# claudiotomasi/LearnMultigrid

Measured on AMD Instinct MI355X. Metric: fine-level DoF*sweeps/s, 2-D Poisson V-cycle, higher is better.
Workload: dtype f64; 1 GPU; 2-D structured P1 Poisson 4096x4096 elements (16785409 DoF, 83861509 nnz, CSR fp64/int32), 6-level V(3,3) cycle, weighted Jacobi omega=0.80, tensor-product geometric transfer, Galerkin RAP by device SpGEMM; mode=vcycle, step=one full V-cycle, hipgraph=True, partition=row blocks of grid lines over 1 rank(s), sweep_variant=0, packed_csr=True, fine_level_format=stencil, problem=poisson, transfer=geometric

## Files before the change

### include/lmg.h

```cpp
#ifndef LMG_H
#define LMG_H

#include <stddef.h>
#include <stdint.h>

#ifdef __cplusplus
extern "C" {
#endif

#define LMG_VERSION 100

typedef enum {
    LMG_OK = 0,
    LMG_ERR_ARG = -1,
    LMG_ERR_ALIGN = -2,
    LMG_ERR_LAUNCH = -3,
    LMG_ERR_CAPACITY = -4,
    LMG_ERR_NODEVICE = -5
} lmg_status;

int lmg_version(void);
const char *lmg_status_string(int status);
int lmg_device_count(void);

// ... 17 lines not shown
int lmg_pcsr_tile_rows(void);
int lmg_pcsr_sweep(int mode, int64_t n, int64_t nnz, int32_t tile_rows, int32_t tile_cap,
                   const int32_t *d_tile_base,
                   const int32_t *d_tile_colbase, const uint8_t *d_rowlen, const void *d_col,
                   int colmode, const void *d_val, int valmode, const double *d_dict, int32_t ndict,
                   const double *d_x, const double *d_b, double *d_out, double alpha, double beta,
                   double *d_partials, double *d_norm2, void *stream);

int lmg_rpat_limits(int32_t *max_patterns, int32_t *max_entries);
int lmg_rpat_sweep(int mode, int64_t n, const uint8_t *d_pid, int32_t npat, int32_t nent, int32_t max_len,
                   const int32_t *d_pat_ptr, const int32_t *d_pat_off, const double *d_pat_val,
                   const double *d_x, const double *d_b, double *d_out, double alpha, double beta,
                   double *d_partials, double *d_norm2, void *stream);
int lmg_rpat_row_hash(int64_t n, const int32_t *d_rowptr, const int32_t *d_colidx, const double *d_vals,
                      uint64_t *d_hash, void *stream);
int lmg_rpat_claim(int64_t n, const uint8_t *d_pid, int32_t *d_rep, void *stream);
int lmg_rpat_verify(int64_t n, int64_t ncols, const int32_t *d_rowptr, const int32_t *d_colidx,
                    const double *d_vals, const uint8_t *d_pid, int32_t npat, const int32_t *d_pat_ptr,
                    const int32_t *d_pat_off, const double *d_pat_val, int32_t *d_mismatch, void *stream);

int lmg_rpat_sweep_grid(int mode, int64_t n, const int32_t *h_grid_map, const uint8_t *d_pid, int32_t npat,
                        int32_t nent, int32_t max_len, const int32_t *d_pat_ptr, const int32_t *d_pat_off,
                        const double *d_pat_val, const double *d_x, const double *d_b, double *d_out,
                        double alpha, double beta, double *d_partials, double *d_norm2, void *stream);
int lmg_rpat_row_hash_grid(int64_t n, const int32_t *h_grid_map, const int32_t *d_rowptr,
                           const int32_t *d_colidx, const double *d_vals, uint64_t *d_hash, void *stream);
int lmg_rpat_verify_grid(int64_t n, int64_t ncols, const int32_t *h_grid_map, const int32_t *d_rowptr,
                         const int32_t *d_colidx, const double *d_vals, const uint8_t *d_pid, int32_t npat,
                         const int32_t *d_pat_ptr, const int32_t *d_pat_off, const double *d_pat_val,
                         int32_t *d_mismatch, void *stream);

int lmg_stencil_limits(int32_t *max_patterns);
int lmg_stencil_sweep(int mode, int64_t n, int32_t line_stride, const uint8_t *d_pid, int32_t npat,
                      const double *d_st_val, const int32_t *d_st_mask, uint32_t union_mask, const double *d_x,
                      const double *d_b, double *d_out, double alpha, double beta, double *d_partials,
                      double *d_norm2, void *stream);

int lmg_stencil_smooth_supported(uint32_t union_mask);
int lmg_stencil_smooth(int64_t n, int32_t line_stride, const uint8_t *d_pid, int32_t npat,
                       const double *d_st_val, const int32_t *d_st_mask, uint32_t union_mask,
                       int32_t hot_pattern, const double *h_hot_val, int sweeps, const double *d_x_in,
                       const double *d_b, double omega, double *d_x_out, double *d_r_out, void *stream);

int lmg_stencil_smooth_tiled_supported(uint32_t union_mask);
int lmg_stencil_smooth_tiled(int64_t n, int32_t line_stride, const uint8_t *d_pid, int32_t npat,
                             const double *d_st_val, const int32_t *d_st_mask, uint32_t union_mask,
                             int32_t hot_pattern, const double *h_hot_val, int sweeps, const double *d_x_in,
                             const double *d_b, double omega, double *d_x_out, double *d_r_out, void *stream);
int lmg_stencil_smooth_tiled_prolong(int64_t n, int32_t line_stride, const uint8_t *d_pid, int32_t npat,
                                     const double *d_st_val, const int32_t *d_st_mask, uint32_t union_mask,
                                     int32_t hot_pattern, const double *h_hot_val, int sweeps, const double *d_x_in,
                                     const double *d_b, double omega, double *d_x_out, int64_t n_coarse,
                                     int32_t coarse_stride, const double *d_e_coarse, const uint8_t *d_p_pid,
                                     int32_t p_npat, const double *d_p_val, const int32_t *d_p_mask, void *stream);
int lmg_stencil_smooth_tiled_restrict(int64_t n, int32_t line_stride, const uint8_t *d_pid, int32_t npat,
                                      const double *d_st_val, const int32_t *d_st_mask, uint32_t union_mask,
                                      int32_t hot_pattern, const double *h_hot_val, int sweeps, const double *d_x_in,
                                      const double *d_b, double omega, double *d_x_out, int64_t n_coarse,
                                      int32_t coarse_stride, double *d_b_coarse, const uint8_t *d_r_pid,
                                      int32_t r_npat, const double *d_r_val, const int32_t *d_r_mask, void *stream);

int lmg_dia_smooth_supported(uint32_t union_mask);
int lmg_dia_fill(int64_t n, int32_t line_stride, const int32_t *d_rowptr, const int32_t *d_colidx, const double *d_vals,
                 uint32_t union_mask, double *d_dia, int32_t *d_mismatch, uint32_t *d_mask_out, void *stream);
int lmg_dia_smooth(int64_t n, int32_t line_stride, uint32_t union_mask, const double *d_dia, int sweeps,
                   const double *d_x_in, const double *d_b, double omega, double *d_x_out, double *d_r_out, void *stream);

int lmg_stencil_smooth_prolong_supported(uint32_t union_mask);
int lmg_stencil_smooth_prolong(int64_t n, int32_t line_stride, const uint8_t *d_pid, int32_t npat,
                               const double *d_st_val, const int32_t *d_st_mask, uint32_t union_mask,
                               int32_t hot_pattern, const double *h_hot_val, int sweeps, const double *d_x_in,
                               const double *d_b, double omega, double *d_x_out, int64_t n_coarse,
                               int32_t coarse_stride, const double *d_e_coarse, const uint8_t *d_p_pid,
                               int32_t p_npat, const double *d_p_val, const int32_t *d_p_mask,
                               const int32_t *h_hot_pairs, const double *h_hot_pval, void *stream);

int lmg_stencil_smooth_restrict(int64_t n, int32_t line_stride, const uint8_t *d_pid, int32_t npat,
                                const double *d_st_val, const int32_t *d_st_mask, uint32_t union_mask,
                                int32_t hot_pattern, const double *h_hot_val, int sweeps, const double *d_x_in,
                                const double *d_b, double omega, double *d_x_out, int64_t n_coarse,
                                int32_t coarse_stride, double *d_b_coarse, const uint8_t *d_r_pid,
                                int32_t r_npat, const double *d_r_val, const int32_t *d_r_mask, int32_t hot_r,
                                const double *h_hot_rval, void *stream);

int lmg_sell_sweep(int mode, int64_t n, const int64_t *d_slice_base, const int32_t *d_slice_len,
                   const int32_t *d_slice_cmin, const int32_t *d_rowlen, const void *d_col, int colmode,
                   const double *d_val, int32_t max_len, const double *d_x, const double *d_b, double *d_out,
                   double alpha, double beta, double *d_partials, double *d_norm2, void *stream);
int lmg_sell_slice_info(int64_t n, const int32_t *d_rowptr, const int32_t *d_colidx, int32_t *d_slice_len,
                        int32_t *d_cmin, int32_t *d_cmax, void *stream);
int lmg_sell_fill(int64_t n, const int32_t *d_rowptr, const int32_t *d_colidx, const double *d_vals,
                  const int64_t *d_slice_base, const int32_t *d_slice_cmin, int colmode, void *d_col_out,
                  double *d_val_out, void *stream);

int lmg_pcsr_tile_colrange(int64_t n, int32_t tile_rows, const int32_t *d_rowptr, const int32_t *d_colidx,
                           int32_t *d_cmin, int32_t *d_cmax, void *stream);
int lmg_pcsr_encode_cols16(int64_t n, int32_t tile_rows, const int32_t *d_rowptr, const int32_t *d_colidx,
                           const int32_t *d_colbase, uint16_t *d_out, void *stream);
int lmg_value_set_collect(const uint64_t *d_table, int64_t table_slots, uint64_t *d_out, int32_t cap, int32_t *d_count,
                          void *stream);
int lmg_value_set_insert(int64_t count, const double *d_vals, uint64_t *d_table, int64_t table_slots,
                         int32_t limit, int32_t *d_state, void *stream);
int lmg_value_encode(int64_t count, const double *d_vals, const double *d_dict, int32_t ndict, int width,
                     void *d_out, int32_t *d_missing, void *stream);
int lmg_csr_inverse_diagonal(int64_t n, const int32_t *d_rowptr, const int32_t *d_colidx, const double *d_vals,
                             double *d_dinv, void *stream);

int lmg_csr_transpose_max_row(void);
int lmg_csr_transpose_count(int64_t nnz, int64_t ncols, const int32_t *d_colidx, int32_t *d_counts, void *stream);
int lmg_csr_transpose_fill(int64_t n, int64_t ncols, const int32_t *d_rowptr, const int32_t *d_colidx,
                           const double *d_vals, const int32_t *d_t_rowptr, int32_t *d_cursor, int32_t *d_t_colidx,
                           double *d_t_vals, void *stream);

// ... 130 lines not shown
```

### learnmultigrid_amd/_lib.py

```python
import ctypes
import os
import subprocess

import torch

_HERE = os.path.dirname(os.path.abspath(__file__))
LIB_PATH = os.environ.get("LMG_LIB_PATH") or os.path.join(_HERE, "liblmg_hip.so")
CSRC = os.path.join(_HERE, "csrc")

_c = ctypes
_i64, _i32, _f64, _p, _cp = _c.c_int64, _c.c_int32, _c.c_double, _c.c_void_p, _c.c_char_p

SIGNATURES = {
    "lmg_version": (_c.c_int, []),
    "lmg_status_string": (_cp, [_c.c_int]),
    "lmg_device_count": (_c.c_int, []),
    "lmg_tune_set": (_c.c_int, [_cp, _c.c_int]),
    "lmg_tune_get": (_c.c_int, [_cp]),
    "lmg_partials_count": (_i64, [_i64]),
    "lmg_csr_residual_norm2": (_c.c_int, [_i64, _i64, _p, _p, _p, _p, _p, _p, _p, _p, _p]),
    "lmg_csr_jacobi": (_c.c_int, [_i64, _i64, _p, _p, _p, _p, _p, _f64, _p, _p]),
    "lmg_csr_spmv": (_c.c_int, [_i64, _i64, _p, _p, _p, _p, _p, _f64, _f64, _p]),
    "lmg_pcsr_tile_rows": (_c.c_int, []),
    "lmg_pcsr_sweep": (_c.c_int, [_c.c_int, _i64, _i64, _i32, _i32, _p, _p, _p, _p, _c.c_int, _p, _c.c_int, _p, _i32,
                                  _p, _p, _p, _f64, _f64, _p, _p, _p]),
    "lmg_rpat_limits": (_c.c_int, [_p, _p]),
    "lmg_rpat_sweep": (_c.c_int, [_c.c_int, _i64, _p, _i32, _i32, _i32, _p, _p, _p, _p, _p, _p, _f64, _f64, _p, _p, _p]),
    "lmg_rpat_row_hash": (_c.c_int, [_i64, _p, _p, _p, _p, _p]),
    "lmg_rpat_claim": (_c.c_int, [_i64, _p, _p, _p]),
    "lmg_rpat_verify": (_c.c_int, [_i64, _i64, _p, _p, _p, _p, _i32, _p, _p, _p, _p, _p]),
    "lmg_rpat_sweep_grid": (_c.c_int, [_c.c_int, _i64, _p, _p, _i32, _i32, _i32, _p, _p, _p, _p, _p, _p, _f64, _f64, _p, _p, _p]),
    "lmg_rpat_row_hash_grid": (_c.c_int, [_i64, _p, _p, _p, _p, _p, _p]),
    "lmg_rpat_verify_grid": (_c.c_int, [_i64, _i64, _p, _p, _p, _p, _p, _i32, _p, _p, _p, _p, _p]),
    "lmg_stencil_limits": (_c.c_int, [_p]),
    "lmg_stencil_sweep": (_c.c_int, [_c.c_int, _i64, _i32, _p, _i32, _p, _p, _c.c_uint32, _p, _p, _p, _f64, _f64, _p, _p, _p]),
    "lmg_stencil_smooth_supported": (_c.c_int, [_c.c_uint32]),
    "lmg_stencil_smooth": (_c.c_int, [_i64, _i32, _p, _i32, _p, _p, _c.c_uint32, _i32, _p, _c.c_int, _p, _p, _f64, _p, _p, _p]),
    "lmg_stencil_smooth_tiled_supported": (_c.c_int, [_c.c_uint32]),
    "lmg_stencil_smooth_tiled": (_c.c_int, [_i64, _i32, _p, _i32, _p, _p, _c.c_uint32, _i32, _p, _c.c_int, _p, _p, _f64, _p, _p, _p]),
    "lmg_stencil_smooth_tiled_prolong": (_c.c_int, [_i64, _i32, _p, _i32, _p, _p, _c.c_uint32, _i32, _p, _c.c_int, _p, _p, _f64, _p,
                                                    _i64, _i32, _p, _p, _i32, _p, _p, _p]),
    "lmg_stencil_smooth_tiled_restrict": (_c.c_int, [_i64, _i32, _p, _i32, _p, _p, _c.c_uint32, _i32, _p, _c.c_int, _p, _p, _f64, _p,
                                                     _i64, _i32, _p, _p, _i32, _p, _p, _p]),
    "lmg_dia_smooth_supported": (_c.c_int, [_c.c_uint32]),
    "lmg_dia_fill": (_c.c_int, [_i64, _i32, _p, _p, _p, _c.c_uint32, _p, _p, _p, _p]),
    "lmg_dia_smooth": (_c.c_int, [_i64, _i32, _c.c_uint32, _p, _c.c_int, _p, _p, _f64, _p, _p, _p]),
    "lmg_stencil_smooth_prolong_supported": (_c.c_int, [_c.c_uint32]),
    "lmg_stencil_smooth_prolong": (_c.c_int, [_i64, _i32, _p, _i32, _p, _p, _c.c_uint32, _i32, _p, _c.c_int, _p, _p, _f64, _p,
                                              _i64, _i32, _p, _p, _i32, _p, _p, _p, _p, _p]),
    "lmg_stencil_smooth_restrict": (_c.c_int, [_i64, _i32, _p, _i32, _p, _p, _c.c_uint32, _i32, _p, _c.c_int, _p, _p, _f64, _p,
                                               _i64, _i32, _p, _p, _i32, _p, _p, _i32, _p, _p]),
    "lmg_sell_sweep": (_c.c_int, [_c.c_int, _i64, _p, _p, _p, _p, _p, _c.c_int, _p, _i32, _p, _p, _p, _f64, _f64, _p, _p, _p]),
    "lmg_sell_slice_info": (_c.c_int, [_i64, _p, _p, _p, _p, _p, _p]),
    "lmg_sell_fill": (_c.c_int, [_i64, _p, _p, _p, _p, _p, _c.c_int, _p, _p, _p]),
    "lmg_pcsr_tile_colrange": (_c.c_int, [_i64, _i32, _p, _p, _p, _p, _p]),
    "lmg_pcsr_encode_cols16": (_c.c_int, [_i64, _i32, _p, _p, _p, _p, _p]),
    "lmg_value_set_collect": (_c.c_int, [_p, _i64, _p, _i32, _p, _p]),
    "lmg_value_set_insert": (_c.c_int, [_i64, _p, _p, _i64, _i32, _p, _p]),
    "lmg_value_encode": (_c.c_int, [_i64, _p, _p, _i32, _c.c_int, _p, _p, _p]),
    "lmg_csr_inverse_diagonal": (_c.c_int, [_i64, _p, _p, _p, _p, _p]),
    "lmg_csr_transpose_max_row": (_c.c_int, []),
    "lmg_csr_transpose_count": (_c.c_int, [_i64, _i64, _p, _p, _p]),
    "lmg_csr_transpose_fill": (_c.c_int, [_i64, _i64, _p, _p, _p, _p, _p, _p, _p, _p]),
    "lmg_csr_gs_rows": (_c.c_int, [_p, _p, _p, _p, _p, _p, _i64, _p]),
    "lmg_csr_gs_schedule": (_c.c_int, [_p, _p, _p, _p, _p, _p, _p, _p, _i64, _i64, _c.c_int, _p]),
    "lmg_csr_gs_schedule_ell": (_c.c_int, [_i64, _p, _p, _p, _p, _p, _p, _p, _i32, _i64, _p, _i64, _c.c_int, _p]),
    "lmg_stencil_gs_supported": (_c.c_int, [_c.c_uint32]),
    "lmg_stencil_gs_work_bytes": (_i64, [_i64, _i32]),
    "lmg_stencil_gs_sweep": (_c.c_int, [_i64, _i32, _p, _i32, _p, _p, _c.c_uint32, _i32, _p, _p, _p, _p, _c.c_int, _p]),
    "lmg_host_gs_levels": (_i64, [_i64, _p, _p, _p]),
    "lmg_host_greedy_colors": (_i64, [_i64, _p, _p, _p]),
    "lmg_axpby": (_c.c_int, [_i64, _f64, _p, _f64, _p, _p]),
    "lmg_vmul": (_c.c_int, [_i64, _f64, _p, _p, _p, _p]),
    "lmg_copy": (_c.c_int, [_i64, _p, _p, _p]),
    "lmg_zero": (_c.c_int, [_i64, _p, _p]),
    "lmg_dot": (_c.c_int, [_i64, _p, _p, _p, _p, _p]),
    "lmg_gather": (_c.c_int, [_i64, _p, _p, _p, _p]),
    "lmg_scatter": (_c.c_int, [_i64, _p, _p, _p, _p]),
    "lmg_dense_gemv": (_c.c_int, [_i64, _i64, _p, _p, _p, _p]),
    "lmg_dense_gemv_blockdiag": (_c.c_int, [_i64, _i64, _p, _p, _p, _p]),
    "lmg_dense_gemv_windows": (_c.c_int, [_i64, _i64, _i64, _p, _p, _i64, _p, _i64, _f64, _p, _i64, _p]),
    "lmg_dense_gemv_windows_off": (_c.c_int, [_i64, _i64, _i64, _p, _p, _p, _p, _i64, _f64, _p, _i64, _p]),
    "lmg_coarse_front": (_c.c_int, [_i64, _i64, _p, _p, _p, _p, _i64, _p, _p]),
    "lmg_coarse_back": (_c.c_int, [_i64, _i64, _i64, _p, _p, _p, _p, _i64, _f64, _p, _p, _c.c_int, _i64, _p]),
    "lmg_coarse_front_gather": (_c.c_int, [_i64, _i64, _p, _p, _p, _p, _i64, _p, _p, _p]),
    "lmg_coarse_back_gather": (_c.c_int, [_i64, _i64, _i64, _p, _p, _p, _p, _i64, _f64, _p, _p, _c.c_int, _i64, _p, _p]),
    "lmg_batched_gemm": (_c.c_int, [_i64, _i64, _i64, _i64, _f64, _p, _i64, _i64, _p, _i64, _i64, _f64, _p, _i64, _i64, _p]),
    "lmg_copy2d": (_c.c_int, [_i64, _i64, _i64, _f64, _p, _i64, _i64, _p, _i64, _i64, _c.c_int, _p]),
    "lmg_pattern_parity_counts": (_c.c_int, [_i64, _i32, _p, _p, _p]),
    "lmg_block_copy": (_c.c_int, [_i64, _i64, _p, _i64, _p, _i64, _p]),
    "lmg_csr_to_dense": (_c.c_int, [_i64, _i64, _p, _p, _p, _p, _p]),
    "lmg_batched_inverse": (_c.c_int, [_i64, _i32, _p, _p, _p, _p]),
    "lmg_spgemm_count": (_c.c_int, [_i64, _p, _p, _p, _p, _p, _p]),
    "lmg_spgemm_symbolic": (_c.c_int, [_i64, _p, _p, _p, _p, _p, _i32, _p, _p]),
    "lmg_spgemm_numeric": (_c.c_int, [_i64, _p, _p, _p, _p, _p, _p, _p, _i32, _p, _p, _p, _p]),
    "lmg_spgemm_numeric_record": (_c.c_int, [_i64, _p, _p, _p, _p, _p, _p, _p, _i32, _p, _p, _p, _p, _p, _p, _p]),
# ... 53 lines not shown
```

### learnmultigrid_amd/csrc/stencil_tile.hip

```cpp
#include <string.h>
#include "lmg_common.hpp"

namespace {

constexpr int kRB = 2;
constexpr int kMaxPat = 64;
constexpr int kCols = 64;
constexpr int kLS = kCols + 2;
constexpr unsigned kMask5 = 0x0BAu;
constexpr unsigned kMask9 = 0x1FFu;

__device__ __forceinline__ double dpp_lower(double src)
{
    const int lo = __builtin_amdgcn_update_dpp(0, __double2loint(src), 0x138, 0xf, 0xf, false);
    const int hi = __builtin_amdgcn_update_dpp(0, __double2hiint(src), 0x138, 0xf, 0xf, false);
    return __hiloint2double(hi, lo);
}
__device__ __forceinline__ double dpp_upper(double src)
{
    const int lo = __builtin_amdgcn_update_dpp(0, __double2loint(src), 0x130, 0xf, 0xf, false);
    const int hi = __builtin_amdgcn_update_dpp(0, __double2hiint(src), 0x130, 0xf, 0xf, false);
    return __hiloint2double(hi, lo);
}

struct __attribute__((aligned(8))) d2u { double a, b; };

struct TArgs {
    int n, W, lines, npat;
    int tiles_x, tiles_y;
    const unsigned char *pid;
    const double *st_val;
    const int *st_mask;
    const double *x;
    const double *b;
    double *out;
    double *r;
    double omega;
    int hot;
    double hot_val[9];
    double hot_rdiag;
    const double *ec;
    int nc, Wc;
    const unsigned char *ppid;
    const double *pp_val;
    const int *pp_mask;
    int pp_npat;
    double *bc;
    const unsigned char *rpid;
    const double *rp_val;
    const int *rp_mask;
    int rp_npat;
};

template <int S, unsigned UM, bool RESID, bool ZERO, int RR, bool PROL = false, bool REST = false, int RBV = kRB>
__global__ void __launch_bounds__(RR / RBV * LMG_WAVE, (RR / RBV == 16 && !PROL) ? 8 : 1) stencil_tile_kernel(TArgs a)
{
    static_assert(!PROL || (!RESID && !ZERO), "the correction is folded into post-smoothing passes only");
    static_assert(!REST || (RESID && !PROL), "the restriction replaces the store of the residual");
    constexpr int H = S + (RESID ? 1 : 0) - (ZERO ? 1 : 0) + (REST ? 1 : 0);
    constexpr int kWaves = RR / RBV, kBlock = kWaves * LMG_WAVE;
    static_assert(RR > 2 * H + 1 && kCols > 2 * H && RR % RBV == 0, "tile smaller than its halo / lines per wave");
    __shared__ double s_x[2][RR * kLS];
    __shared__ double s_val[kMaxPat * 9];
    __shared__ int s_mask[kMaxPat];
    __shared__ double s_rdiag[kMaxPat];
    __shared__ double s_pv[PROL ? kMaxPat * 4 : 1];
    __shared__ int s_pm[PROL ? kMaxPat : 1];
    __shared__ double s_rv[REST ? kMaxPat * 9 : 1];
    __shared__ int s_rm[REST ? kMaxPat : 1];

    const int t = threadIdx.x, lane = t & (LMG_WAVE - 1), wave = t >> 6;
    const int tx = (int)blockIdx.x % a.tiles_x, ty = (int)blockIdx.x / a.tiles_x;
    const int c0 = tx * (kCols - 2 * H) - H, y0 = ty * (RR - 2 * H) - H;
    const int n = a.n;
    const int64_t W = a.W;
    constexpr int RB = RBV;
    constexpr bool DIAG = (UM & 0x145u) != 0;
    const int rb0 = wave * RB;

    double lx[RB], bk[RB];
    int pk[RB];
    double le[PROL ? RB : 1][4];
    int lq[(PROL || REST) ? RB : 1];
#pragma unroll
    for (int k = 0; k < RB; ++k) {
        const int y = y0 + rb0 + k;
        const int64_t i = (int64_t)y * W + c0 + lane;
        const bool ok = y >= 0 && y < a.lines && i >= 0 && i < n;
        const int64_t j = ok ? i : 0;
        lx[k] = (!ZERO && ok) ? a.x[j] : 0.0;
        bk[k] = ok ? a.b[j] : 0.0;
        pk[k] = ok ? ((int)a.pid[j] | 0x100) : 0;
        if (PROL) {
            const int c = c0 + lane;
            int yy, xx;
            if (a.W >= 2 * kCols) {
                yy = c < 0 ? y - 1 : (c >= a.W ? y + 1 : y);
                xx = c < 0 ? c + a.W : (c >= a.W ? c - a.W : c);
            } else {
                yy = (int)((unsigned)j / (unsigned)a.W);
                xx = (int)((unsigned)j - (unsigned)yy * (unsigned)a.W);
            }
            const int64_t base = (int64_t)(yy >> 1) * a.Wc + (xx >> 1);
            lq[k] = ok ? (int)a.ppid[j] : 0;
            const int64_t b0 = ok ? min(base, (int64_t)a.nc - 2) : 0, b1 = ok ? min(base + a.Wc, (int64_t)a.nc - 2) : 0;
            const d2u e01 = *reinterpret_cast<const d2u *>(a.ec + b0), e23 = *reinterpret_cast<const d2u *>(a.ec + b1);
            le[k][0] = b0 == base ? e01.a : e01.b;
            le[k][1] = e01.b;
            le[k][2] = b1 == base + a.Wc ? e23.a : e23.b;
            le[k][3] = e23.b;
        }
        if (REST) {
            const int c = c0 + lane;
            const bool crow = ok && !(y & 1) && !(c & 1) && c >= 0 && c < W;
            const int64_t jc = (int64_t)(y >> 1) * a.Wc + (c >> 1);
            lq[k] = crow ? ((int)a.rpid[jc < a.nc ? jc : 0] | 0x100) : 0;
        }
    }
    for (int i = t; i < a.npat * 9; i += kBlock) s_val[i] = a.st_val[i];
    for (int i = t; i < a.npat; i += kBlock) {
        const int m = a.st_mask[i];
        const double dg = (m & 16) ? a.st_val[i * 9 + 4] : 0.0;
        s_rdiag[i] = dg != 0.0 ? 1.0 / dg : 0.0;
        s_mask[i] = dg == 0.0 ? (m | (1 << 16)) : m;
    }
    for (int i = t; i < 2 * RR; i += kBlock) {
        const int r = i >> 1, g = (i & 1) ? kLS - 1 : 0;
        s_x[0][r * kLS + g] = 0.0;
        s_x[1][r * kLS + g] = 0.0;
    }
    if (PROL) {
        for (int i = t; i < a.pp_npat * 4; i += kBlock) s_pv[i] = a.pp_val[i];
        for (int i = t; i < a.pp_npat; i += kBlock) s_pm[i] = a.pp_mask[i];
        __syncthreads();
#pragma unroll
        for (int k = 0; k < RB; ++k) {
            const int m = s_pm[lq[k]];
            double acc = 0.0;
#pragma unroll
            for (int q = 0; q < 4; ++q) {
                const double tv = acc + s_pv[lq[k] * 4 + q] * le[k][q];
                acc = ((m >> q) & 1) ? tv : acc;
            }
            lx[k] = (pk[k] >> 8) ? lx[k] + acc : 0.0;
        }
    }
    if (REST) {
        for (int i = t; i < a.rp_npat * 9; i += kBlock) s_rv[i] = a.rp_val[i];
        for (int i = t; i < a.rp_npat; i += kBlock) s_rm[i] = a.rp_mask[i];
    }
    const int hot = a.hot >= 0 ? (a.hot | 0x100) : -1;
    bool mine = true;
#pragma unroll
    for (int k = 0; k < RB; ++k) {
        s_x[0][(rb0 + k) * kLS + 1 + lane] = lx[k];
        s_x[1][(rb0 + k) * kLS + 1 + lane] = 0.0;
        mine = mine && (pk[k] == hot || !(pk[k] >> 8));
    }
    const bool all_hot = __all(mine);
    __syncthreads();

    const double omega = a.omega;
    double hv[9];
#pragma unroll
    for (int s = 0; s < 9; ++s) hv[s] = a.hot_val[s];
    const double hrd = a.hot_rdiag;

    struct Win { double m, c, p; };
    auto line = [&](const double *src, int r, bool sides) -> Win {
        Win w;
        w.c = src[r * kLS + 1 + lane];
        w.m = sides ? dpp_lower(w.c) : 0.0;
        w.p = sides ? dpp_upper(w.c) : 0.0;
        return w;
    };
    auto apply = [&](const Win &u, const Win &c, const Win &d, int p, bool hotp) -> double {
        const double w[9] = {u.m, u.c, u.p, c.m, c.c, c.p, d.m, d.c, d.p};
        double acc = 0.0;
        if (hotp) {
#pragma unroll
            for (int s = 0; s < 9; ++s)
                if ((UM >> s) & 1u) acc = acc + hv[s] * w[s];
        } else {
            const int q = p & 0xff, m = s_mask[q];
// ... 12 lines not shown
        for (int j = 0; j < RB + 2; ++j) {
            const int rr = min(max(rb0 - 1 + j, 0), RR - 1);
            ln[j] = line(src, rr, DIAG || (j >= 1 && j <= RB));
        }
        if (all_hot) {
#pragma unroll
            for (int k = 0; k < RB; ++k) {
                const double acc = apply(ln[k], ln[k + 1], ln[k + 2], pk[k], true);
                emit(k, rb0 + k >= lo && rb0 + k < hi, true, ln[k + 1].c, acc);
            }
        } else {
#pragma unroll
            for (int k = 0; k < RB; ++k) {
                const double acc = apply(ln[k], ln[k + 1], ln[k + 2], pk[k], false);
                emit(k, rb0 + k >= lo && rb0 + k < hi, false, ln[k + 1].c, acc);
            }
        }
    };

#pragma unroll
    for (int s = 1; s <= S; ++s) {
        const double *src = s_x[(s - 1) & 1];
        double *dst = s_x[s & 1];
        if (ZERO && s == 1) {
#pragma unroll
            for (int k = 0; k < RB; ++k)
                dst[(rb0 + k) * kLS + 1 + lane] = (pk[k] >> 8) ? omega * (s_rdiag[pk[k] & 0xff] * bk[k]) : 0.0;
        } else {
            block(src, 1, RR - 1, [&](int k, bool keep, bool hotp, double xc, double acc) {
                const double res = bk[k] - acc;
                double nx;
                if (hotp) {
                    nx = xc + omega * (hrd * res);
                } else {
                    const int q = pk[k] & 0xff;
                    nx = (s_mask[q] >> 16) ? xc : xc + omega * (s_rdiag[q] * res);
                }
                if (keep) dst[(rb0 + k) * kLS + 1 + lane] = (pk[k] >> 8) ? nx : 0.0;
            });
        }
        __syncthreads();
    }

    const double *fin = s_x[S & 1];
    const bool col_ok = lane >= H && lane < kCols - H && c0 + lane >= 0 && c0 + lane < W;
    if (REST) {
        double *rl = s_x[(S + 1) & 1];
        block(fin, 1, RR - 1, [&](int k, bool keep, bool, double xc, double acc) {
            const int r = rb0 + k;
            if (keep) rl[r * kLS + 1 + lane] = bk[k] - acc;
            if (r >= H && r < RR - H && col_ok && (pk[k] >> 8)) a.out[(int64_t)(y0 + r) * W + c0 + lane] = xc;
        });
        __syncthreads();
#pragma unroll
        for (int k = 0; k < RB; ++k) {
            const int r = rb0 + k;
            const int q = lq[k] & 0xff, m = s_rm[q];
            double acc = 0.0;
#pragma unroll
            for (int e = 0; e < 9; ++e) {
                const int rr = min(max(r + e / 3 - 1, 0), RR - 1);
                const double tv = acc + s_rv[q * 9 + e] * rl[rr * kLS + 1 + lane + e % 3 - 1];
                acc = ((m >> e) & 1) ? tv : acc;
            }
            if ((lq[k] >> 8) && r >= H && r < RR - H && col_ok)
                a.bc[(int64_t)((y0 + r) >> 1) * a.Wc + ((c0 + lane) >> 1)] = acc;
        }
    } else if (RESID) {
        block(fin, H, RR - H, [&](int k, bool keep, bool, double xc, double acc) {
            const int64_t i = (int64_t)(y0 + rb0 + k) * W + c0 + lane;
            if (keep && col_ok && (pk[k] >> 8)) {
                a.out[i] = xc;
                a.r[i] = bk[k] - acc;
            }
        });
    } else {
#pragma unroll
        for (int k = 0; k < RB; ++k) {
            const int r = rb0 + k;
            if (r >= H && r < RR - H && col_ok && (pk[k] >> 8))
                a.out[(int64_t)(y0 + r) * W + c0 + lane] = fin[r * kLS + 1 + lane];
        }
    }
}

int g_tile_rows = 16;
int g_tile_prol_wide_lines = 768;
int g_tile_rows_big = 0;
int g_tile_big_lines = 600;

template <int S, unsigned UM, bool RESID, bool ZERO, int RR, bool PROL = false, bool REST = false, int RBV = kRB>
int launch5(TArgs a, hipStream_t st)
{
    constexpr int H = S + (RESID ? 1 : 0) - (ZERO ? 1 : 0) + (REST ? 1 : 0);
    a.tiles_x = (a.W + (kCols - 2 * H) - 1) / (kCols - 2 * H);
    a.tiles_y = (a.lines + (RR - 2 * H) - 1) / (RR - 2 * H);
    const int64_t grid = (int64_t)a.tiles_x * a.tiles_y;
    if (grid > 0x7fffffff) return LMG_ERR_CAPACITY;
    hipLaunchKernelGGL((stencil_tile_kernel<S, UM, RESID, ZERO, RR, PROL, REST, RBV>), dim3((unsigned)grid), dim3(RR / RBV * LMG_WAVE), 0, st,
                       a);
    LMG_CHECK_LAUNCH();
    return LMG_OK;
}

static int tile_rows_for(const TArgs &a)
{
    const int rr = a.lines >= g_tile_big_lines ? g_tile_rows_big : g_tile_rows;
    return rr == 0 ? 32 : rr;
}

template <int S, unsigned UM, bool RESID, bool ZERO, bool PROL = false, bool REST = false>
int launch4(TArgs a, hipStream_t st)
{
    if (tile_rows_for(a) == 16) return launch5<S, UM, RESID, ZERO, 16, PROL, REST>(a, st);
    if constexpr (PROL) {
        if (a.lines >= g_tile_prol_wide_lines) return launch5<S, UM, RESID, ZERO, 32, PROL, REST, 4>(a, st);
    }
    return launch5<S, UM, RESID, ZERO, 32, PROL, REST>(a, st);
}

template <unsigned UM>
int launch_prol(TArgs a, int sweeps, hipStream_t st)
{
    switch (sweeps) {
    case 1: return launch4<1, UM, false, false, true>(a, st);
    case 2: return launch4<2, UM, false, false, true>(a, st);
    default: return launch4<3, UM, false, false, true>(a, st);
    }
}

template <unsigned UM>
int launch_rest(TArgs a, int sweeps, bool zero, hipStream_t st)
{
    switch (sweeps) {
    case 1: return zero ? launch4<1, UM, true, true, false, true>(a, st) : launch4<1, UM, true, false, false, true>(a, st);
    case 2: return zero ? launch4<2, UM, true, true, false, true>(a, st) : launch4<2, UM, true, false, false, true>(a, st);
    default: return zero ? launch4<3, UM, true, true, false, true>(a, st) : launch4<3, UM, true, false, false, true>(a, st);
    }
}

template <int S, unsigned UM>
int launch2(TArgs a, bool resid, bool zero, hipStream_t st)
{
    if (resid) return zero ? launch4<S, UM, true, true>(a, st) : launch4<S, UM, true, false>(a, st);
    return zero ? launch4<S, UM, false, true>(a, st) : launch4<S, UM, false, false>(a, st);
}

template <unsigned UM>
int launch1(TArgs a, int sweeps, bool resid, bool zero, hipStream_t st)
{
    switch (sweeps) {
    case 1: return launch2<1, UM>(a, resid, zero, st);
    case 2: return launch2<2, UM>(a, resid, zero, st);
    default: return launch2<3, UM>(a, resid, zero, st);
    }
}

}

int lmg_tile_tune_set(const char *key, int v)
{
    if (strcmp(key, "tile_rows") == 0 || strcmp(key, "tile_rows_big") == 0) {
        if (v != 0 && v != 16 && v != 32) return LMG_ERR_ARG;
        (key[9] ? g_tile_rows_big : g_tile_rows) = v;
        return LMG_OK;
    }
    if (strcmp(key, "tile_prol_wide_lines") == 0) {
        if (v < 0) return LMG_ERR_ARG;
        g_tile_prol_wide_lines = v;
        return LMG_OK;
    }
    if (strcmp(key, "tile_big_lines") == 0) {
        if (v < 0) return LMG_ERR_ARG;
        g_tile_big_lines = v;
        return LMG_OK;
    }
    return LMG_ERR_ARG;
}
int lmg_tile_tune_get(const char *key)
{
    if (strcmp(key, "tile_rows") == 0) return g_tile_rows;
    if (strcmp(key, "tile_rows_big") == 0) return g_tile_rows_big;
    if (strcmp(key, "tile_big_lines") == 0) return g_tile_big_lines;
    if (strcmp(key, "tile_prol_wide_lines") == 0) return g_tile_prol_wide_lines;
    return LMG_ERR_ARG;
}

extern "C" {

static int tile_args(TArgs &a, int64_t n, int32_t line_stride, const uint8_t *pid, int32_t npat, const double *st_val,
                     const int32_t *st_mask, uint32_t union_mask, int32_t hot_pattern, const double *h_hot_val, int sweeps,
                     const double *x_in, const double *b, double omega, double *x_out, double *r_out)
{
    if (n < 0 || n >= (1ll << 31) - 4096 || npat < 1 || npat > kMaxPat || (union_mask & ~0x1FFu)) return LMG_ERR_ARG;
    if (sweeps < 1 || sweeps > 3) return LMG_ERR_ARG;
    if (n == 0) return LMG_OK;
    if (!pid || !st_val || !st_mask || !b || !x_out || x_in == x_out || r_out == x_out || (r_out && r_out == x_in))
        return LMG_ERR_ARG;
    if (line_stride < 3 || line_stride > n) return LMG_ERR_ARG;
    a.n = (int)n;
    a.W = line_stride;
    a.lines = (int)((n + line_stride - 1) / line_stride);
    a.npat = npat;
    a.tiles_x = a.tiles_y = 0;
    a.pid = pid;
    a.st_val = st_val;
    a.st_mask = st_mask;
    a.x = x_in;
    a.b = b;
    a.out = x_out;
    a.r = r_out;
    a.omega = omega;
    a.hot = -1;
    for (int k = 0; k < 9; ++k) a.hot_val[k] = 0.0;
    a.hot_rdiag = 0.0;
    if (hot_pattern >= 0 && hot_pattern < npat && h_hot_val && h_hot_val[4] != 0.0) {
        a.hot = hot_pattern;
        for (int k = 0; k < 9; ++k) a.hot_val[k] = h_hot_val[k];
        a.hot_rdiag = 1.0 / h_hot_val[4];
    }
    a.ec = nullptr;
    a.nc = a.Wc = 0;
    a.ppid = nullptr;
    a.pp_val = nullptr;
    a.pp_mask = nullptr;
    a.pp_npat = 0;
    a.bc = nullptr;
    a.rpid = nullptr;
    a.rp_val = nullptr;
    a.rp_mask = nullptr;
    a.rp_npat = 0;
    return 1;
}

int lmg_stencil_smooth_tiled(int64_t n, int32_t line_stride, const uint8_t *pid, int32_t npat, const double *st_val,
                             const int32_t *st_mask, uint32_t union_mask, int32_t hot_pattern, const double *h_hot_val,
                             int sweeps, const double *x_in, const double *b, double omega, double *x_out, double *r_out,
                             void *stream)
{
    TArgs a;
    const int rc = tile_args(a, n, line_stride, pid, npat, st_val, st_mask, union_mask, hot_pattern, h_hot_val, sweeps, x_in, b,
                             omega, x_out, r_out);
    if (rc != 1) return rc;
    hipStream_t st = lmg_stream(stream);
    const bool resid = r_out != nullptr, zero = x_in == nullptr;
    switch (union_mask) {
    case kMask5: return launch1<kMask5>(a, sweeps, resid, zero, st);
    case kMask9: return launch1<kMask9>(a, sweeps, resid, zero, st);
    default: return LMG_ERR_CAPACITY;
    }
}

int lmg_stencil_smooth_tiled_prolong(int64_t n, int32_t line_stride, const uint8_t *pid, int32_t npat, const double *st_val,
                                     const int32_t *st_mask, uint32_t union_mask, int32_t hot_pattern,
                                     const double *h_hot_val, int sweeps, const double *x_in, const double *b, double omega,
                                     double *x_out, int64_t n_coarse, int32_t coarse_stride, const double *e_coarse,
                                     const uint8_t *p_pid, int32_t p_npat, const double *p_val, const int32_t *p_mask,
                                     void *stream)
{
    if (!x_in || !e_coarse || !p_pid || !p_val || !p_mask || p_npat < 1 || p_npat > kMaxPat) return LMG_ERR_ARG;
    if (n_coarse < 2 || n_coarse >= (1ll << 31) || coarse_stride < 1 || coarse_stride > n_coarse) return LMG_ERR_ARG;
    if (e_coarse == x_out) return LMG_ERR_ARG;
    TArgs a;
    const int rc = tile_args(a, n, line_stride, pid, npat, st_val, st_mask, union_mask, hot_pattern, h_hot_val, sweeps, x_in, b,
                             omega, x_out, nullptr);
    if (rc != 1) return rc;
    a.ec = e_coarse;
    a.nc = (int)n_coarse;
    a.Wc = coarse_stride;
    a.ppid = p_pid;
    a.pp_val = p_val;
    a.pp_mask = p_mask;
    a.pp_npat = p_npat;
    hipStream_t st = lmg_stream(stream);
    switch (union_mask) {
    case kMask5: return launch_prol<kMask5>(a, sweeps, st);
    case kMask9: return launch_prol<kMask9>(a, sweeps, st);
    default: return LMG_ERR_CAPACITY;
    }
}

int lmg_stencil_smooth_tiled_restrict(int64_t n, int32_t line_stride, const uint8_t *pid, int32_t npat, const double *st_val,
                                      const int32_t *st_mask, uint32_t union_mask, int32_t hot_pattern,
                                      const double *h_hot_val, int sweeps, const double *x_in, const double *b, double omega,
                                      double *x_out, int64_t n_coarse, int32_t coarse_stride, double *b_coarse,
                                      const uint8_t *r_pid, int32_t r_npat, const double *r_val, const int32_t *r_mask,
                                      void *stream)
{
    if (!b_coarse || !r_pid || !r_val || !r_mask || r_npat < 1 || r_npat > kMaxPat) return LMG_ERR_ARG;
    if (n_coarse < 1 || n_coarse >= (1ll << 31) || coarse_stride < 1 || coarse_stride > n_coarse) return LMG_ERR_ARG;
    if ((const double *)b_coarse == x_in || b_coarse == x_out || (const double *)b_coarse == b) return LMG_ERR_ARG;
    const int64_t lines = n > 0 ? (n + line_stride - 1) / line_stride : 0;
    if ((int64_t)coarse_stride != ((int64_t)line_stride + 1) / 2 || (n % line_stride) != 0 || n_coarse != ((lines + 1) / 2) * coarse_stride)
        return LMG_ERR_ARG;
    TArgs a;
    const int rc = tile_args(a, n, line_stride, pid, npat, st_val, st_mask, union_mask, hot_pattern, h_hot_val, sweeps, x_in, b,
                             omega, x_out, nullptr);
    if (rc != 1) return rc;
    a.bc = b_coarse;
    a.nc = (int)n_coarse;
    a.Wc = coarse_stride;
    a.rpid = r_pid;
    a.rp_val = r_val;
    a.rp_mask = r_mask;
    a.rp_npat = r_npat;
    hipStream_t st = lmg_stream(stream);
    const bool zero = x_in == nullptr;
    switch (union_mask) {
    case kMask5: return launch_rest<kMask5>(a, sweeps, zero, st);
    case kMask9: return launch_rest<kMask9>(a, sweeps, zero, st);
    default: return LMG_ERR_CAPACITY;
    }
}

int lmg_stencil_smooth_tiled_supported(uint32_t union_mask)
{
    return union_mask == kMask5 || union_mask == kMask9;
}

}
```

### learnmultigrid_amd/ops.py

```python
import ctypes
import math

import numpy as np
import torch

from . import _lib
from ._lib import LmgError, check

F64 = torch.float64
I32 = torch.int32


def _s(*ts):
    for t in ts:
        if t is not None and getattr(t, "is_cuda", False):
            if t.device.index != torch.cuda.current_device():
                raise LmgError("operands live on %s but the current device is cuda:%d: wrap the call in "
                               "torch.cuda.device(...)" % (t.device, torch.cuda.current_device()))
            return torch.cuda.current_stream(t.device).cuda_stream
    return torch.cuda.current_stream().cuda_stream


def _p(t):
    return None if t is None else t.data_ptr()
# ... 697 lines not shown
_TILED_ENABLED = True


def set_tiled_enabled(flag):
    global _TILED_ENABLED
    _TILED_ENABLED = bool(flag)


def _fused_kind(A):
    S = getattr(A, "stencil", None)
    D = getattr(A, "dia", None)
    if S is None and D is not None and _PACKED_ENABLED and _DIA_ENABLED and _FUSED_ENABLED:
        return "dia"
    if not (_PACKED_ENABLED and _STENCIL_ENABLED and _FUSED_ENABLED and S is not None):
        return None
    if S.n >= FUSED_MIN_ROWS:
        return "reg" if (S.n < REG_MAX_ROWS and _lib.lib().lmg_stencil_smooth_supported(S.umask)) else None
    if _TILED_ENABLED and S.n >= TILED_MIN_ROWS and S.W >= 3 and _lib.lib().lmg_stencil_smooth_tiled_supported(S.umask):
        return "tile"
    return None


def stencil_smooth_available(A):
    return _fused_kind(A) is not None


_FUSED_ENABLED = True


def set_fused_enabled(flag):
    global _FUSED_ENABLED
    _FUSED_ENABLED = bool(flag)


def stencil_smooth(A, x_in, b, omega, sweeps, x_out, r_out=None, prolong=None, restrict=None):
    _vec_ok(x_in, b, x_out, r_out)
    S = A.stencil
    if S is None and getattr(A, "dia", None) is not None:
        D = A.dia
        if prolong is not None or restrict is not None:
            raise LmgError("stencil_smooth: transfers cannot be fused into the pass of a variable-coefficient operator")
        check(_lib.lib().lmg_dia_smooth(D.n, D.W, D.umask, _p(D.dia), int(sweeps), _p(x_in), _p(b), float(omega), _p(x_out),
                                        _p(r_out), _s(D.dia)), "lmg_dia_smooth")
        return
    if S is None:
        raise LmgError("stencil_smooth needs a grid-stencil matrix")
    hv = None if S._hot_val is None else ctypes.addressof(S._hot_val)
    if restrict is not None:
        R, bc = restrict
        T = R.restrict
        _vec_ok(bc)
        if T is None or r_out is not None or prolong is not None or T.n != S.n or T.W != S.W or bc.numel() != T.nc:
            raise LmgError("stencil_smooth: this restriction cannot be fused into the pass")
        if _fused_kind(A) == "tile" and not (S.n >= REG_RESTRICT_MIN_ROWS and _lib.lib().lmg_stencil_smooth_prolong_supported(S.umask)):
            check(_lib.lib().lmg_stencil_smooth_tiled_restrict(S.n, S.W, _p(S.pid), S.npat, _p(S.st_val), _p(S.st_mask), S.umask,
                                                               S.hot, hv, int(sweeps), _p(x_in), _p(b), float(omega), _p(x_out),
                                                               T.nc, T.Wc, _p(bc), _p(T.pid), T.npat, _p(T.r_val), _p(T.r_mask),
                                                               _s(S.pid)), "lmg_stencil_smooth_tiled_restrict")
            return
        hr = None if T._hot_val is None else ctypes.addressof(T._hot_val)
        check(_lib.lib().lmg_stencil_smooth_restrict(S.n, S.W, _p(S.pid), S.npat, _p(S.st_val), _p(S.st_mask), S.umask, S.hot,
                                                     hv, int(sweeps), _p(x_in), _p(b), float(omega), _p(x_out), T.nc, T.Wc,
                                                     _p(bc), _p(T.pid), T.npat, _p(T.r_val), _p(T.r_mask), T.hot, hr, _s(S.pid)),
              "lmg_stencil_smooth_restrict")
        return
    if prolong is not None:
        P, e = prolong
        T = P.prolong
        _vec_ok(e)
        if T is None or r_out is not None or x_in is None or T.n != S.n or T.W != S.W or e.numel() != T.nc:
            raise LmgError("stencil_smooth: this prolongation cannot be fused into the pass")
        if _fused_kind(A) == "tile" and not (S.n >= REG_PROLONG_MIN_ROWS and _lib.lib().lmg_stencil_smooth_prolong_supported(S.umask)):
            check(_lib.lib().lmg_stencil_smooth_tiled_prolong(S.n, S.W, _p(S.pid), S.npat, _p(S.st_val), _p(S.st_mask), S.umask,
                                                              S.hot, hv, int(sweeps), _p(x_in), _p(b), float(omega), _p(x_out),
                                                              T.nc, T.Wc, _p(e), _p(T.pid), T.npat, _p(T.p_val), _p(T.p_mask),
                                                              _s(S.pid)), "lmg_stencil_smooth_tiled_prolong")
            return
        check(_lib.lib().lmg_stencil_smooth_prolong(S.n, S.W, _p(S.pid), S.npat, _p(S.st_val), _p(S.st_mask), S.umask, S.hot,
                                                    hv, int(sweeps), _p(x_in), _p(b), float(omega), _p(x_out), T.nc, T.Wc,
                                                    _p(e), _p(T.pid), T.npat, _p(T.p_val), _p(T.p_mask),
                                                    ctypes.addressof(T._hot_pairs), ctypes.addressof(T._hot_pval), _s(S.pid)),
              "lmg_stencil_smooth_prolong")
        return
    if _fused_kind(A) == "tile":
        check(_lib.lib().lmg_stencil_smooth_tiled(S.n, S.W, _p(S.pid), S.npat, _p(S.st_val), _p(S.st_mask), S.umask, S.hot,
                                                  hv, int(sweeps), _p(x_in), _p(b), float(omega), _p(x_out), _p(r_out), _s(S.pid)),
              "lmg_stencil_smooth_tiled")
        return
    check(_lib.lib().lmg_stencil_smooth(S.n, S.W, _p(S.pid), S.npat, _p(S.st_val), _p(S.st_mask), S.umask, S.hot, hv,
                                        int(sweeps), _p(x_in), _p(b), float(omega), _p(x_out), _p(r_out), _s(S.pid)),
          "lmg_stencil_smooth")


FUSED_TRANSFER_MIN_ROWS = 12_000_000
REG_PROLONG_MIN_ROWS = 1 << 62
REG_RESTRICT_MIN_ROWS = 1 << 62
_FUSED_PROLONG_ENABLED = True


def set_fused_prolong_enabled(flag):
    global _FUSED_PROLONG_ENABLED
    _FUSED_PROLONG_ENABLED = bool(flag)


def stencil_smooth_prolong_available(A, P):
    T = getattr(P, "prolong", None)
    S = getattr(A, "stencil", None)
    kind = _fused_kind(A)
    if not (_FUSED_PROLONG_ENABLED and T is not None and kind in ("reg", "tile") and T.n == S.n and T.W == S.W):
        return False
    if kind == "tile":
        return True
    return bool(S.n >= FUSED_TRANSFER_MIN_ROWS and _lib.lib().lmg_stencil_smooth_prolong_supported(S.umask))


_FUSED_RESTRICT_ENABLED = True
TILED_RESTRICT_MAX_ROWS = 1 << 62


def set_fused_restrict_enabled(flag):
    global _FUSED_RESTRICT_ENABLED
    _FUSED_RESTRICT_ENABLED = bool(flag)


def stencil_smooth_restrict_available(A, R):
    T = getattr(R, "restrict", None)
    S = getattr(A, "stencil", None)
    kind = _fused_kind(A)
# ... 704 lines not shown
```

Before: 249.1 billion DoF*sweeps/s.

## Add hot-pattern fast paths for fused prolongation and restriction in tiled smoother

Adds an HX variant of the tiled stencil kernel. When every lane in a wave hits the dominant pattern, prolongation and restriction weights come from kernel arguments instead of shared-memory pattern tables. Prolongation is folded straight into lx at load time, and restriction assigns one thread per coarse node of the tile instead of the per-line residual path. This is meant to cut shared-memory table loads, syncs and occupancy limits, but it changes the launch bounds, adds wave-uniform branches, and the tiled path only runs for smaller levels where it is selected over the register path.

```diff
diff --git a/include/lmg.h b/include/lmg.h
--- a/include/lmg.h
+++ b/include/lmg.h
@@ -93,13 +93,15 @@
                                      int32_t hot_pattern, const double *h_hot_val, int sweeps, const double *d_x_in,
                                      const double *d_b, double omega, double *d_x_out, int64_t n_coarse,
                                      int32_t coarse_stride, const double *d_e_coarse, const uint8_t *d_p_pid,
-                                     int32_t p_npat, const double *d_p_val, const int32_t *d_p_mask, void *stream);
+                                     int32_t p_npat, const double *d_p_val, const int32_t *d_p_mask,
+                                     const int32_t *h_hot_pairs, const double *h_hot_pval, void *stream);
 int lmg_stencil_smooth_tiled_restrict(int64_t n, int32_t line_stride, const uint8_t *d_pid, int32_t npat,
                                       const double *d_st_val, const int32_t *d_st_mask, uint32_t union_mask,
                                       int32_t hot_pattern, const double *h_hot_val, int sweeps, const double *d_x_in,
                                       const double *d_b, double omega, double *d_x_out, int64_t n_coarse,
                                       int32_t coarse_stride, double *d_b_coarse, const uint8_t *d_r_pid,
-                                      int32_t r_npat, const double *d_r_val, const int32_t *d_r_mask, void *stream);
+                                      int32_t r_npat, const double *d_r_val, const int32_t *d_r_mask, int32_t hot_r,
+                                      const double *h_hot_rval, void *stream);
 
 int lmg_dia_smooth_supported(uint32_t union_mask);
 int lmg_dia_fill(int64_t n, int32_t line_stride, const int32_t *d_rowptr, const int32_t *d_colidx, const double *d_vals,
diff --git a/learnmultigrid_amd/_lib.py b/learnmultigrid_amd/_lib.py
--- a/learnmultigrid_amd/_lib.py
+++ b/learnmultigrid_amd/_lib.py
@@ -39,9 +39,9 @@
     "lmg_stencil_smooth_tiled_supported": (_c.c_int, [_c.c_uint32]),
     "lmg_stencil_smooth_tiled": (_c.c_int, [_i64, _i32, _p, _i32, _p, _p, _c.c_uint32, _i32, _p, _c.c_int, _p, _p, _f64, _p, _p, _p]),
     "lmg_stencil_smooth_tiled_prolong": (_c.c_int, [_i64, _i32, _p, _i32, _p, _p, _c.c_uint32, _i32, _p, _c.c_int, _p, _p, _f64, _p,
-                                                    _i64, _i32, _p, _p, _i32, _p, _p, _p]),
+                                                    _i64, _i32, _p, _p, _i32, _p, _p, _p, _p, _p]),
     "lmg_stencil_smooth_tiled_restrict": (_c.c_int, [_i64, _i32, _p, _i32, _p, _p, _c.c_uint32, _i32, _p, _c.c_int, _p, _p, _f64, _p,
-                                                     _i64, _i32, _p, _p, _i32, _p, _p, _p]),
+                                                     _i64, _i32, _p, _p, _i32, _p, _p, _i32, _p, _p]),
     "lmg_dia_smooth_supported": (_c.c_int, [_c.c_uint32]),
     "lmg_dia_fill": (_c.c_int, [_i64, _i32, _p, _p, _p, _c.c_uint32, _p, _p, _p, _p]),
     "lmg_dia_smooth": (_c.c_int, [_i64, _i32, _c.c_uint32, _p, _c.c_int, _p, _p, _f64, _p, _p, _p]),
diff --git a/learnmultigrid_amd/csrc/stencil_tile.hip b/learnmultigrid_amd/csrc/stencil_tile.hip
--- a/learnmultigrid_amd/csrc/stencil_tile.hip
+++ b/learnmultigrid_amd/csrc/stencil_tile.hip
@@ -50,22 +50,28 @@
     const double *rp_val;
     const int *rp_mask;
     int rp_npat;
+    int phot[2];
+    double phv[9];
+    int rhot;
+    double rhv[9];
 };
 
-template <int S, unsigned UM, bool RESID, bool ZERO, int RR, bool PROL = false, bool REST = false, int RBV = kRB>
-__global__ void __launch_bounds__(RR / RBV * LMG_WAVE, (RR / RBV == 16 && !PROL) ? 8 : 1) stencil_tile_kernel(TArgs a)
+template <int S, unsigned UM, bool RESID, bool ZERO, int RR, bool PROL = false, bool REST = false, int RBV = kRB, bool HX = false>
+__global__ void __launch_bounds__(RR / RBV * LMG_WAVE, (RR / RBV == 16 && (!PROL || HX)) ? 8 : 1) stencil_tile_kernel(TArgs a)
 {
     static_assert(!PROL || (!RESID && !ZERO), "the correction is folded into post-smoothing passes only");
     static_assert(!REST || (RESID && !PROL), "the restriction replaces the store of the residual");
     constexpr int H = S + (RESID ? 1 : 0) - (ZERO ? 1 : 0) + (REST ? 1 : 0);
     constexpr int kWaves = RR / RBV, kBlock = kWaves * LMG_WAVE;
     static_assert(RR > 2 * H + 1 && kCols > 2 * H && RR % RBV == 0, "tile smaller than its halo / lines per wave");
+    static_assert(!HX || PROL || REST, "hot transfers need a transfer");
+    static_assert(!(REST && HX) || (RR - 2 * H + 1) / 2 <= RR / RBV * 2, "a thread per coarse node of the tile");
     __shared__ double s_x[2][RR * kLS];
     __shared__ double s_val[kMaxPat * 9];
     __shared__ int s_mask[kMaxPat];
     __shared__ double s_rdiag[kMaxPat];
-    __shared__ double s_pv[PROL ? kMaxPat * 4 : 1];
-    __shared__ int s_pm[PROL ? kMaxPat : 1];
+    __shared__ double s_pv[(PROL && !HX) ? kMaxPat * 4 : 1];
+    __shared__ int s_pm[(PROL && !HX) ? kMaxPat : 1];
     __shared__ double s_rv[REST ? kMaxPat * 9 : 1];
     __shared__ int s_rm[REST ? kMaxPat : 1];
 
@@ -80,8 +86,19 @@
 
     double lx[RB], bk[RB];
     int pk[RB];
-    double le[PROL ? RB : 1][4];
+    double le[(PROL && !HX) ? RB : 1][4];
     int lq[(PROL || REST) ? RB : 1];
+    int rq = 0, rrow = H, rcol = H;
+    bool rown = false;
+    if (REST && HX) {
+        const int ye0 = (y0 + H + 1) & ~1, xe0 = (c0 + H + 1) & ~1;
+        const int yf = ye0 + 2 * (t >> 5), xf = xe0 + 2 * (t & 31);
+        rown = yf < y0 + RR - H && yf < a.lines && xf < c0 + kCols - H && xf < W;
+        const int64_t jc = (int64_t)(yf >> 1) * a.Wc + (xf >> 1);
+        rq = (rown && jc < a.nc) ? (int)a.rpid[jc] : 0;
+        rrow = rown ? yf - y0 : H;
+        rcol = rown ? xf - c0 : H;
+    }
 #pragma unroll
     for (int k = 0; k < RB; ++k) {
         const int y = y0 + rb0 + k;
@@ -105,12 +122,40 @@
             lq[k] = ok ? (int)a.ppid[j] : 0;
             const int64_t b0 = ok ? min(base, (int64_t)a.nc - 2) : 0, b1 = ok ? min(base + a.Wc, (int64_t)a.nc - 2) : 0;
             const d2u e01 = *reinterpret_cast<const d2u *>(a.ec + b0), e23 = *reinterpret_cast<const d2u *>(a.ec + b1);
-            le[k][0] = b0 == base ? e01.a : e01.b;
-            le[k][1] = e01.b;
-            le[k][2] = b1 == base + a.Wc ? e23.a : e23.b;
-            le[k][3] = e23.b;
-        }
-        if (REST) {
+            const double w0 = b0 == base ? e01.a : e01.b, w1 = e01.b, w2 = b1 == base + a.Wc ? e23.a : e23.b, w3 = e23.b;
+            if (!HX) {
+                le[k][0] = w0;
+                le[k][1] = w1;
+                le[k][2] = w2;
+                le[k][3] = w3;
+            } else {
+                const int yl = yy & 1, xl = xx & 1;
+                const int hp = a.phot[yl];
+                const bool hotk = !ok || (hp >= 0 && lq[k] == ((xl ? hp >> 8 : hp) & 0xff));
+                double acc = 0.0;
+                if (__all(hotk)) {
+                    const double v0 = yl ? (xl ? a.phv[5] : a.phv[3]) : (xl ? a.phv[1] : a.phv[0]);
+                    const double v1 = yl ? a.phv[6] : a.phv[2], v2 = xl ? a.phv[7] : a.phv[4];
+                    acc = acc + v0 * w0;
+                    double tv = acc + v1 * w1;
+                    acc = xl ? tv : acc;
+                    tv = acc + v2 * w2;
+                    acc = yl ? tv : acc;
+                    tv = acc + a.phv[8] * w3;
+                    acc = (xl & yl) ? tv : acc;
+                } else {
+                    const int q = lq[k], m = a.pp_mask[q];
+                    const double w[4] = {w0, w1, w2, w3};
+#pragma unroll
+                    for (int s = 0; s < 4; ++s) {
+                        const double tv = acc + a.pp_val[q * 4 + s] * w[s];
+                        acc = ((m >> s) & 1) ? tv : acc;
+                    }
+                }
+                lx[k] = (pk[k] >> 8) ? lx[k] + acc : 0.0;
+            }
+        }
+        if (REST && !HX) {
             const int c = c0 + lane;
             const bool crow = ok && !(y & 1) && !(c & 1) && c >= 0 && c < W;
             const int64_t jc = (int64_t)(y >> 1) * a.Wc + (c >> 1);
@@ -129,7 +174,7 @@
         s_x[0][r * kLS + g] = 0.0;
         s_x[1][r * kLS + g] = 0.0;
     }
-    if (PROL) {
+    if (PROL && !HX) {
         for (int i = t; i < a.pp_npat * 4; i += kBlock) s_pv[i] = a.pp_val[i];
         for (int i = t; i < a.pp_npat; i += kBlock) s_pm[i] = a.pp_mask[i];
         __syncthreads();
@@ -248,6 +293,25 @@
             if (r >= H && r < RR - H && col_ok && (pk[k] >> 8)) a.out[(int64_t)(y0 + r) * W + c0 + lane] = xc;
         });
         __syncthreads();
+        if (HX) {
+            if (__any(rown)) {
+                const double *p = rl + rrow * kLS + 1 + rcol;
+                double acc = 0.0;
+                if (__all(!rown || rq == a.rhot)) {
+#pragma unroll
+                    for (int e = 0; e < 9; ++e) acc = acc + a.rhv[e] * p[(e / 3 - 1) * kLS + e % 3 - 1];
+                } else {
+                    const int m = s_rm[rq];
+#pragma unroll
+                    for (int e = 0; e < 9; ++e) {
+                        const double tv = acc + s_rv[rq * 9 + e] * p[(e / 3 - 1) * kLS + e % 3 - 1];
+                        acc = ((m >> e) & 1) ? tv : acc;
+                    }
+                }
+                if (rown) a.bc[(int64_t)((y0 + rrow) >> 1) * a.Wc + ((c0 + rcol) >> 1)] = acc;
+            }
+            return;
+        }
 #pragma unroll
         for (int k = 0; k < RB; ++k) {
             const int r = rb0 + k;
@@ -284,8 +348,10 @@
 int g_tile_prol_wide_lines = 768;
 int g_tile_rows_big = 0;
 int g_tile_big_lines = 600;
-
-template <int S, unsigned UM, bool RESID, bool ZERO, int RR, bool PROL = false, bool REST = false, int RBV = kRB>
+int g_tile_hot_transfers = 1;
+int g_tile_prol_wide_lines_hx = 1 << 30;
+
+template <int S, unsigned UM, bool RESID, bool ZERO, int RR, bool PROL = false, bool REST = false, int RBV = kRB, bool HX = false>
 int launch5(TArgs a, hipStream_t st)
 {
     constexpr int H = S + (RESID ? 1 : 0) - (ZERO ? 1 : 0) + (REST ? 1 : 0);
@@ -293,8 +359,8 @@
     a.tiles_y = (a.lines + (RR - 2 * H) - 1) / (RR - 2 * H);
     const int64_t grid = (int64_t)a.tiles_x * a.tiles_y;
     if (grid > 0x7fffffff) return LMG_ERR_CAPACITY;
-    hipLaunchKernelGGL((stencil_tile_kernel<S, UM, RESID, ZERO, RR, PROL, REST, RBV>), dim3((unsigned)grid), dim3(RR / RBV * LMG_WAVE), 0, st,
-                       a);
+    hipLaunchKernelGGL((stencil_tile_kernel<S, UM, RESID, ZERO, RR, PROL, REST, RBV, HX>), dim3((unsigned)grid),
+                       dim3(RR / RBV * LMG_WAVE), 0, st, a);
     LMG_CHECK_LAUNCH();
     return LMG_OK;
 }
@@ -305,14 +371,24 @@
     return rr == 0 ? 32 : rr;
 }
 
+template <int S, unsigned UM, bool RESID, bool ZERO, bool PROL, bool REST, bool HX>
+int launch4x(TArgs a, hipStream_t st)
+{
+    if (tile_rows_for(a) == 16) return launch5<S, UM, RESID, ZERO, 16, PROL, REST, kRB, HX>(a, st);
+    if constexpr (PROL) {
+        if (a.lines >= (HX ? g_tile_prol_wide_lines_hx : g_tile_prol_wide_lines))
+            return launch5<S, UM, RESID, ZERO, 32, PROL, REST, 4, HX>(a, st);
+    }
+    return launch5<S, UM, RESID, ZERO, 32, PROL, REST, kRB, HX>(a, st);
+}
+
 template <int S, unsigned UM, bool RESID, bool ZERO, bool PROL = false, bool REST = false>
 int launch4(TArgs a, hipStream_t st)
 {
-    if (tile_rows_for(a) == 16) return launch5<S, UM, RESID, ZERO, 16, PROL, REST>(a, st);
-    if constexpr (PROL) {
-        if (a.lines >= g_tile_prol_wide_lines) return launch5<S, UM, RESID, ZERO, 32, PROL, REST, 4>(a, st);
-    }
-    return launch5<S, UM, RESID, ZERO, 32, PROL, REST>(a, st);
+    if constexpr (PROL || REST) {
+        if (g_tile_hot_transfers) return launch4x<S, UM, RESID, ZERO, PROL, REST, true>(a, st);
+    }
+    return launch4x<S, UM, RESID, ZERO, PROL, REST, false>(a, st);
 }
 
 template <unsigned UM>
@@ -361,9 +437,9 @@
         (key[9] ? g_tile_rows_big : g_tile_rows) = v;
         return LMG_OK;
     }
-    if (strcmp(key, "tile_prol_wide_lines") == 0) {
+    if (strcmp(key, "tile_prol_wide_lines") == 0 || strcmp(key, "tile_prol_wide_lines_hx") == 0) {
         if (v < 0) return LMG_ERR_ARG;
-        g_tile_prol_wide_lines = v;
+        (key[20] ? g_tile_prol_wide_lines_hx : g_tile_prol_wide_lines) = v;
         return LMG_OK;
     }
     if (strcmp(key, "tile_big_lines") == 0) {
@@ -371,6 +447,11 @@
         g_tile_big_lines = v;
         return LMG_OK;
     }
+    if (strcmp(key, "tile_hot_transfers") == 0) {
+        if (v != 0 && v != 1) return LMG_ERR_ARG;
+        g_tile_hot_transfers = v;
+        return LMG_OK;
+    }
     return LMG_ERR_ARG;
 }
 int lmg_tile_tune_get(const char *key)
@@ -379,6 +460,8 @@
     if (strcmp(key, "tile_rows_big") == 0) return g_tile_rows_big;
     if (strcmp(key, "tile_big_lines") == 0) return g_tile_big_lines;
     if (strcmp(key, "tile_prol_wide_lines") == 0) return g_tile_prol_wide_lines;
+    if (strcmp(key, "tile_hot_transfers") == 0) return g_tile_hot_transfers;
+    if (strcmp(key, "tile_prol_wide_lines_hx") == 0) return g_tile_prol_wide_lines_hx;
     return LMG_ERR_ARG;
 }
 
@@ -426,6 +509,9 @@
     a.rp_val = nullptr;
     a.rp_mask = nullptr;
     a.rp_npat = 0;
+    a.phot[0] = a.phot[1] = -1;
+    a.rhot = -1;
+    for (int k = 0; k < 9; ++k) a.phv[k] = a.rhv[k] = 0.0;
     return 1;
 }
 
@@ -452,7 +538,7 @@
                                      const double *h_hot_val, int sweeps, const double *x_in, const double *b, double omega,
                                      double *x_out, int64_t n_coarse, int32_t coarse_stride, const double *e_coarse,
                                      const uint8_t *p_pid, int32_t p_npat, const double *p_val, const int32_t *p_mask,
-                                     void *stream)
+                                     const int32_t *h_hot_pairs, const double *h_hot_pval, void *stream)
 {
     if (!x_in || !e_coarse || !p_pid || !p_val || !p_mask || p_npat < 1 || p_npat > kMaxPat) return LMG_ERR_ARG;
     if (n_coarse < 2 || n_coarse >= (1ll << 31) || coarse_stride < 1 || coarse_stride > n_coarse) return LMG_ERR_ARG;
@@ -468,6 +554,14 @@
     a.pp_val = p_val;
     a.pp_mask = p_mask;
     a.pp_npat = p_npat;
+    if (h_hot_pairs && h_hot_pval) {
+        for (int k = 0; k < 2; ++k) {
+            const int hp = h_hot_pairs[k];
+            const bool ok = hp >= 0 && (hp & 0xff) < p_npat && (hp >> 8) < p_npat;
+            a.phot[k] = ok ? hp : -1;
+        }
+        for (int k = 0; k < 9; ++k) a.phv[k] = h_hot_pval[k];
+    }
     hipStream_t st = lmg_stream(stream);
     switch (union_mask) {
     case kMask5: return launch_prol<kMask5>(a, sweeps, st);
@@ -481,7 +575,7 @@
                                       const double *h_hot_val, int sweeps, const double *x_in, const double *b, double omega,
                                       double *x_out, int64_t n_coarse, int32_t coarse_stride, double *b_coarse,
                                       const uint8_t *r_pid, int32_t r_npat, const double *r_val, const int32_t *r_mask,
-                                      void *stream)
+                                      int32_t hot_r, const double *h_hot_rval, void *stream)
 {
     if (!b_coarse || !r_pid || !r_val || !r_mask || r_npat < 1 || r_npat > kMaxPat) return LMG_ERR_ARG;
     if (n_coarse < 1 || n_coarse >= (1ll << 31) || coarse_stride < 1 || coarse_stride > n_coarse) return LMG_ERR_ARG;
@@ -500,6 +594,10 @@
     a.rp_val = r_val;
     a.rp_mask = r_mask;
     a.rp_npat = r_npat;
+    if (hot_r >= 0 && hot_r < r_npat && h_hot_rval) {
+        a.rhot = hot_r;
+        for (int k = 0; k < 9; ++k) a.rhv[k] = h_hot_rval[k];
+    }
     hipStream_t st = lmg_stream(stream);
     const bool zero = x_in == nullptr;
     switch (union_mask) {
diff --git a/learnmultigrid_amd/ops.py b/learnmultigrid_amd/ops.py
--- a/learnmultigrid_amd/ops.py
+++ b/learnmultigrid_amd/ops.py
@@ -773,13 +773,13 @@
         _vec_ok(bc)
         if T is None or r_out is not None or prolong is not None or T.n != S.n or T.W != S.W or bc.numel() != T.nc:
             raise LmgError("stencil_smooth: this restriction cannot be fused into the pass")
+        hr = None if T._hot_val is None else ctypes.addressof(T._hot_val)
         if _fused_kind(A) == "tile" and not (S.n >= REG_RESTRICT_MIN_ROWS and _lib.lib().lmg_stencil_smooth_prolong_supported(S.umask)):
             check(_lib.lib().lmg_stencil_smooth_tiled_restrict(S.n, S.W, _p(S.pid), S.npat, _p(S.st_val), _p(S.st_mask), S.umask,
                                                                S.hot, hv, int(sweeps), _p(x_in), _p(b), float(omega), _p(x_out),
                                                                T.nc, T.Wc, _p(bc), _p(T.pid), T.npat, _p(T.r_val), _p(T.r_mask),
-                                                               _s(S.pid)), "lmg_stencil_smooth_tiled_restrict")
+                                                               T.hot, hr, _s(S.pid)), "lmg_stencil_smooth_tiled_restrict")
             return
-        hr = None if T._hot_val is None else ctypes.addressof(T._hot_val)
         check(_lib.lib().lmg_stencil_smooth_restrict(S.n, S.W, _p(S.pid), S.npat, _p(S.st_val), _p(S.st_mask), S.umask, S.hot,
                                                      hv, int(sweeps), _p(x_in), _p(b), float(omega), _p(x_out), T.nc, T.Wc,
                                                      _p(bc), _p(T.pid), T.npat, _p(T.r_val), _p(T.r_mask), T.hot, hr, _s(S.pid)),
@@ -795,6 +795,7 @@
             check(_lib.lib().lmg_stencil_smooth_tiled_prolong(S.n, S.W, _p(S.pid), S.npat, _p(S.st_val), _p(S.st_mask), S.umask,
                                                               S.hot, hv, int(sweeps), _p(x_in), _p(b), float(omega), _p(x_out),
                                                               T.nc, T.Wc, _p(e), _p(T.pid), T.npat, _p(T.p_val), _p(T.p_mask),
+                                                              ctypes.addressof(T._hot_pairs), ctypes.addressof(T._hot_pval),
                                                               _s(S.pid)), "lmg_stencil_smooth_tiled_prolong")
             return
         check(_lib.lib().lmg_stencil_smooth_prolong(S.n, S.W, _p(S.pid), S.npat, _p(S.st_val), _p(S.st_mask), S.umask, S.hot,
```

After: 259.6 billion DoF*sweeps/s (median of 6 runs). 1.04x the previous value.
